# monahand1023/imageclust

Measured on AMD Instinct MI355X. Metric: images/sec (embed+Ward), higher is better.
Workload: dtype bf16; 1 GPU; the metric's size (configs[2]'s N=100000) on 1 GPU: 100000 synthetic 224x224x3 images (structured, seed 20250217; 100000 on this rank), ResNet50-v1 bf16 batch=256 -> 2048-d pooled E -> Ward min=5 max=50 (merge loop on GPU0) -> cluster ids on host; n_images_total=100000, embed_dim=2048, weights=synthetic seed 1, device=AMD Radeon Graphics (gfx950:sramecc+:xnack-)

## Files before the change

imageclust_amd/csrc/resnet.hip:

```cpp
#include "icl_common.h"
#include "jpeg_stage.h"
#include "mfma_tile.h"

#include <algorithm>
#include <cmath>
#include <chrono>
#include <condition_variable>
#include <cstring>
#include <new>
#include <thread>
#include <type_traits>
#include <vector>

#define ICL_MAX_LANES 4

struct conv_args {
    const void *X;
    const void *Wt;
    void *Y;
    const void *R;
    const float *scale;
    const float *shift;
    const void *zero;
    int B, H, W, Cin, Ho, Wo, Cout, KH, KW, stride, pad, relu;
// ... 1142 lines not shown
            ICL_HIP(ctx, hipMemcpy(*dst, t.data(), n * 2, hipMemcpyHostToDevice));
        } else if (prec == ICL_PREC_BF16X3) {
            std::vector<uint16_t> t(2 * n);
            host_split32(src, n, t.data());
            ICL_HIP(ctx, hipMemcpy(*dst, t.data(), n * 4, hipMemcpyHostToDevice));
        } else {
            ICL_HIP(ctx, hipMemcpy(*dst, src, n * 4, hipMemcpyHostToDevice));
        }
        return ICL_OK;
    };
    void *dx = nullptr, *dw = nullptr, *dr = nullptr, *dy = nullptr, *dz = nullptr;
    float *dsc = nullptr, *dsh = nullptr;
    int rc = to_dev(x, nx, &dx);
    if (!rc && (hipMalloc(&dz, 256) != hipSuccess || hipMemset(dz, 0, 256) != hipSuccess)) rc = icl_fail(ctx, ICL_ERR_NOMEM, "icl_conv2d_fused: zero page");
    if (!rc) rc = to_dev(wp.data(), nw, &dw);
    if (!rc && residual) rc = to_dev(residual, ny, &dr);
    if (!rc) rc = upload(ctx, (void **)&dsc, scale, (size_t)Cout * 4);
    if (!rc) rc = upload(ctx, (void **)&dsh, shift, (size_t)Cout * 4);
    if (!rc && hipMalloc(&dy, ny * es) != hipSuccess) rc = icl_fail(ctx, ICL_ERR_NOMEM, "icl_conv2d_fused: output alloc");
    if (!rc) {
        conv_args a;
        a.X = dx; a.Wt = dw; a.Y = dy; a.R = dr; a.scale = dsc; a.shift = dsh; a.zero = dz;
        a.X2 = nullptr; a.H2 = a.W2 = a.Cin2 = a.stride2 = 0;
        a.B = B; a.H = a.W = H; a.Cin = Cin; a.Ho = a.Wo = Ho; a.Cout = Cout; a.KH = a.KW = k; a.stride = stride; a.pad = pad;
        a.relu = relu; a.M = (int64_t)B * Ho * Ho; a.K = k * k * Cin;
        rc = launch_conv_prec(ctx, prec, a);
    }
    if (!rc) {
        hipError_t e = hipStreamSynchronize(ctx->stream);
        if (e == hipSuccess) {
            if (prec == ICL_PREC_BF16) {
                std::vector<uint16_t> t(ny);
                e = hipMemcpy(t.data(), dy, ny * 2, hipMemcpyDeviceToHost);
                for (size_t i = 0; i < ny; ++i) y[i] = host_from_bf16(t[i]);
            } else if (prec == ICL_PREC_BF16X3) {
                std::vector<uint16_t> t(2 * ny);
                e = hipMemcpy(t.data(), dy, ny * 4, hipMemcpyDeviceToHost);
                host_join32(t.data(), ny, y);
            } else {
                e = hipMemcpy(y, dy, ny * 4, hipMemcpyDeviceToHost);
            }
        }
        if (e != hipSuccess) rc = icl_fail(ctx, ICL_ERR_HIP, "icl_conv2d_fused: %s", hipGetErrorString(e));
    }
    for (void *q : {dx, dw, dr, dy, dz, (void *)dsc, (void *)dsh})
        if (q) (void)hipFree(q);
    icl_prof_collect(ctx);
    return rc;
}

static int launch_conv_fused_ds(icl_ctx *ctx, int prec, const conv_layer &c3, const conv_layer &ds, const void *t2, const void *x, void *y, int B)
{
    conv_args a;
    a.X = t2;
    a.Wt = c3.wfused[prec];
    a.Y = y;
    a.R = nullptr;
    a.scale = ctx->model->ones;
    a.shift = c3.shift_fused;
    a.zero = ctx->model->zero;
    a.B = B;
    a.relu = 1;
    a.Cout = c3.rec.cout;
    a.H = a.W = a.Ho = a.Wo = c3.rec.hout;
    a.Cin = c3.rec.cin;
    a.KH = a.KW = 1;
    a.stride = 1;
    a.pad = 0;
    a.X2 = x;
    a.H2 = a.W2 = ds.rec.hin;
    a.Cin2 = ds.rec.cin;
    a.stride2 = ds.rec.stride;
    a.M = (int64_t)B * a.Ho * a.Wo;
    a.K = a.Cin + a.Cin2;
    const int bk = prec == ICL_PREC_BF16 ? BF16::BK : F32::BK;
    if (a.Cin % bk || a.Cin2 % bk || a.Cout % 128) return icl_fail(ctx, ICL_ERR_UNSUPPORTED, "fused downsample shape not supported");
    return launch_conv_prec(ctx, prec, a);
}

static int fuse_mask()
{
    static const int m = [] {
        const char *e = getenv("ICL_FUSE");
        return e ? atoi(e) : 15;
    }();
    return m;
}

template <typename T>
static void launch_stem_pool(icl_ctx *ctx, int prec, const uint8_t *d_img, int B, void *pooled, hipStream_t strm)
{
    icl_model *m = ctx->model;
    if (prec == ICL_PREC_BF16 && (fuse_mask() & 8)) {
        const conv_layer &L0 = m->conv[0];
        icl_prof_scope ps(ctx, ICL_K_CONV64, 2.0 * (double)B * 112 * 112 * 64 * 147, 0.0);
        const int nunits = B * SP_STRIPS;
        const int per_cu = std::max<int>(1, std::min<int>(5, (int)((size_t)160 * 1024 / stem2_lds_bytes())));
        const unsigned grid = (unsigned)std::min<int64_t>(nunits, (int64_t)per_cu * ctx->prop.multiProcessorCount);
        hipLaunchKernelGGL(stem2_pool_kernel, dim3(grid), dim3(256), stem2_lds_bytes(), strm, d_img, (const uint16_t *)L0.wfold, L0.shift, (uint16_t *)pooled, nunits);
        return;
    }
    constexpr bool SPLIT = is_x3<T>::value;
    typedef typename std::conditional<SPLIT, F32, T>::type TS;
    icl_lds_optin(ctx, (const void *)stem_pool_kernel<TS, SPLIT>, (int)stem_pool_lds_bytes<TS>());
    conv_args a;
    const conv_layer &L = m->conv[0];
    a.X = nullptr; a.Wt = L.w[SPLIT ? ICL_PREC_FP32 : prec]; a.Y = pooled; a.R = nullptr; a.scale = L.scale; a.shift = L.shift; a.zero = m->zero;
    a.B = B; a.H = a.W = 224; a.Cin = 3; a.Ho = a.Wo = 112; a.Cout = 64; a.KH = a.KW = 7; a.stride = 2; a.pad = 3; a.relu = 1;
    a.M = (int64_t)B * 112 * 112; a.K = STEM_K; a.gx = B * SP_STRIPS * SP_TILES; a.gy = 1;
    a.X2 = nullptr; a.H2 = a.W2 = a.Cin2 = a.stride2 = 0;
    icl_prof_scope ps(ctx, ICL_K_CONV64, 2.0 * (double)a.M * 64 * 147, 0.0);
    const int nunits = B * SP_STRIPS;
    const int per_cu = std::max<int>(1, (int)((size_t)160 * 1024 / stem_pool_lds_bytes<TS>()));
    const unsigned grid = (unsigned)std::min<int64_t>(nunits, (int64_t)per_cu * ctx->prop.multiProcessorCount);
    hipLaunchKernelGGL((stem_pool_kernel<TS, SPLIT>), dim3(grid), dim3(256), stem_pool_lds_bytes<TS>(), strm, d_img, a, nunits);
}

static int launch_bneck56(icl_ctx *ctx, const conv_layer &c1, const conv_layer &c2, const conv_layer &c3, const conv_layer *ds, const void *x, void *y,
                          int B, hipStream_t strm)
{
    bneck_args a;
    a.X = (const uint16_t *)x;
    a.Y = (uint16_t *)y;
    a.W1 = (const uint16_t *)c1.wfold;
    a.W2 = (const uint16_t *)c2.wfold;
    a.W3 = (const uint16_t *)(ds ? c3.wfused[ICL_PREC_BF16] : c3.wfold);
    a.sh1 = c1.shift; a.sh2 = c2.shift;
    a.sh3 = ds ? c3.shift_fused : c3.shift;
    a.B = B; a.H = c2.rec.hin; a.W = c2.rec.hin;
    if ((int64_t)B * a.H * a.W * 512 >= (1LL << 31)) return icl_fail(ctx, ICL_ERR_UNSUPPORTED, "fused bottleneck: batch of %d images exceeds the 32-bit buffer offsets", B);
    a.nstrips = (a.W + BN56_COLS - 1) / BN56_COLS;
    a.ngroups = std::max(1, std::min(B, ctx->prop.multiProcessorCount / a.nstrips));
#ifdef BN56_TIMERS
    static unsigned long long *dbg = nullptr;
    if (!dbg) (void)hipMalloc((void **)&dbg, 16 * 8);
    a.dbg = dbg;
#endif
    const double px = (double)B * a.H * a.W;
    icl_prof_scope ps(ctx, ICL_K_CONV, 2.0 * px * (64.0 * c1.rec.cin + 64.0 * 576 + 256.0 * (ds ? 128 : 64)), 0.0);
    const dim3 grid((unsigned)(a.nstrips * a.ngroups));
    if (ds) {
        icl_lds_optin(ctx, (const void *)bneck56_kernel<true>, (int)bneck56_lds_bytes<true>());
        hipLaunchKernelGGL((bneck56_kernel<true>), grid, dim3(512), bneck56_lds_bytes<true>(), strm, a);
    } else {
        icl_lds_optin(ctx, (const void *)bneck56_kernel<false>, (int)bneck56_lds_bytes<false>());
        hipLaunchKernelGGL((bneck56_kernel<false>), grid, dim3(512), bneck56_lds_bytes<false>(), strm, a);
    }
    ICL_HIP(ctx, hipGetLastError());
#ifdef BN56_TIMERS
    if (getenv("BN56_PRINT")) {
        unsigned long long h[16];
        (void)hipStreamSynchronize(strm);
        (void)hipMemcpy(h, dbg, sizeof h, hipMemcpyDeviceToHost);
        const char *fn[8] = {"carry+conv1", "wait E", "dma+t1 epi", "wait C", "conv2+t2 epi", "wait x", "wait D", ""};
        const char *bn[8] = {"t2 reads + side wait", "ST reads + t2 MFMAs", "DMA issue", "side MFMAs + epilogue", "read-back + stores", "barrier waits", "", ""};
        const int nsteps = ((B / a.ngroups) * (a.H + 1) + 7) / 8;
        fprintf(stderr, "[bn56 %s] cycles per step (steps %d):\n  front:", ds ? "ds" : "id", nsteps);
        for (int k = 0; k < 7; ++k) fprintf(stderr, " %s %.0f |", fn[k], (double)h[k] / nsteps);
        fprintf(stderr, "\n  back :");
        for (int k = 0; k < 7; ++k) fprintf(stderr, " %s %.0f |", bn[k], (double)h[8 + k] / nsteps);
        fprintf(stderr, "\n");
    }
#endif
    return ICL_OK;
}

template <typename T>
static int forward_batch(icl_ctx *ctx, int prec, const uint8_t *d_img, int B, int head, float *d_out, int lane, hipStream_t strm)
{
    typedef typename T::elem elem;
    icl_model *m = ctx->model;
    ctx->cur_stream = strm;
    const int grid = 256 * 8;
    elem *x = (elem *)m->buf[lane][0], *t1 = (elem *)m->buf[lane][1], *t2 = (elem *)m->buf[lane][2], *ds = (elem *)m->buf[lane][3],
         *y = (elem *)m->buf[lane][4];
    if ((fuse_mask() & 1) || is_x3<T>::value) {
        launch_stem_pool<T>(ctx, prec, d_img, B, x, strm);
    } else if constexpr (!is_x3<T>::value) {
        {
            icl_lds_optin(ctx, (const void *)stem_conv_kernel<T>, (int)stem_lds_bytes<T>());
            conv_args a;
            const conv_layer &L = m->conv[0];
            a.X = nullptr; a.Wt = L.w[prec]; a.Y = y; a.R = nullptr; a.scale = L.scale; a.shift = L.shift; a.zero = m->zero;
            a.B = B; a.H = a.W = 224; a.Cin = 3; a.Ho = a.Wo = 112; a.Cout = 64; a.KH = a.KW = 7; a.stride = 2; a.pad = 3; a.relu = 1;
            a.M = (int64_t)B * 112 * 112; a.K = STEM_K; a.gx = B * 98; a.gy = 1;
            a.X2 = nullptr; a.H2 = a.W2 = a.Cin2 = a.stride2 = 0;
            icl_prof_scope ps(ctx, ICL_K_CONV64, 2.0 * (double)a.M * 64 * 147, 0.0);
            const int per_cu = std::max<int>(1, (int)((size_t)160 * 1024 / stem_lds_bytes<T>()));
            const unsigned stem_grid = (unsigned)std::min<int64_t>(a.gx, (int64_t)per_cu * ctx->prop.multiProcessorCount);
            hipLaunchKernelGGL((stem_conv_kernel<T>), dim3(stem_grid), dim3(256), stem_lds_bytes<T>(), strm, d_img, a);
        }
        {
            icl_prof_scope ps(ctx, ICL_K_EMBED_OTHER, 0.0, (double)B * (802816.0 + 200704.0) * sizeof(elem));
            hipLaunchKernelGGL((maxpool_kernel<T>), dim3(grid), dim3(256), 0, strm, y, B, 112, 64, x);
        }
    }
    int ci = 1;
    while (ci < m->nconv) {
        const conv_layer &c1 = m->conv[ci], &c2 = m->conv[ci + 1], &c3 = m->conv[ci + 2];
        const bool has_ds = c1.rec.block == 0;
        if (prec == ICL_PREC_BF16 && c1.rec.stage == 1 && (fuse_mask() & (has_ds ? 4 : 2))) {
            ICL_TRY(launch_bneck56(ctx, c1, c2, c3, has_ds ? &m->conv[ci + 3] : nullptr, x, y, B, strm));
            std::swap(x, y);
            ci += has_ds ? 4 : 3;
            continue;
        }
        ICL_TRY(launch_conv(ctx, prec, c1, x, t1, nullptr, 1, B));
        ICL_TRY(launch_conv(ctx, prec, c2, t1, t2, nullptr, 1, B));
        if (has_ds)
            ICL_TRY(launch_conv_fused_ds(ctx, prec, c3, m->conv[ci + 3], t2, x, y, B));
        else
            ICL_TRY(launch_conv(ctx, prec, c3, t2, y, x, 1, B));
        std::swap(x, y);
        ci += has_ds ? 4 : 3;
    }
    float *pooled = head == ICL_HEAD_POOLED ? d_out : m->pooled[lane];
    {
        icl_prof_scope ps(ctx, ICL_K_EMBED_OTHER, 0.0, (double)B * 49.0 * 2048.0 * (is_x3<T>::value ? 4 : sizeof(elem)));
        hipLaunchKernelGGL((avgpool_kernel<T>), dim3((unsigned)icl_ceil_div((int64_t)B * 2048, 256)), dim3(256), 0, strm, x, B, 49,
                           ICL_FEAT_DIM, pooled, (int64_t)ICL_FEAT_DIM);
    }
    if (head == ICL_HEAD_DENSE0) {
        icl_prof_scope ps(ctx, ICL_K_EMBED_OTHER, 2.0 * B * 2048.0 * 1000.0, 0.0);
        hipLaunchKernelGGL(fc_kernel, dim3((unsigned)std::min<int64_t>(icl_ceil_div((int64_t)B * ICL_FC_OUT, 4), 4096)), dim3(256), 0,
                           strm, pooled, m->fcw, m->fcb, B, ICL_FEAT_DIM, ICL_FC_OUT, d_out);
    }
    ICL_HIP(ctx, hipGetLastError());
    return ICL_OK;
}

extern "C" int icl_stem_pool(icl_ctx *ctx, int prec, const uint8_t *img, int B, float *out)
{
    if (!ctx || !img || !out || B < 1) return icl_fail(ctx, ICL_ERR_ARG, "icl_stem_pool: bad argument");
    if (!prec_ok(prec)) return icl_fail(ctx, ICL_ERR_ARG, "bad prec");
    return no_throw(ctx, "icl_stem_pool", [&]() -> int {
        std::lock_guard<std::mutex> lk(ctx->mu);
        icl_device_guard g(ctx->device);
        if (!ctx->model) return icl_fail(ctx, ICL_ERR_NOMODEL, "no model loaded (call icl_model_load_* first)");
        const size_t es = prec == ICL_PREC_BF16 ? 2 : 4, ny = (size_t)B * 56 * 56 * 64;
        uint8_t *dimg = nullptr;
        void *dy = nullptr;
        int rc = ICL_OK;
        if (hipMalloc((void **)&dimg, (size_t)B * ICL_IMG_BYTES) != hipSuccess || hipMalloc(&dy, ny * es) != hipSuccess)
            rc = icl_fail(ctx, ICL_ERR_NOMEM, "icl_stem_pool: device buffers");
        if (!rc && hipMemcpy(dimg, img, (size_t)B * ICL_IMG_BYTES, hipMemcpyHostToDevice) != hipSuccess) rc = icl_fail(ctx, ICL_ERR_HIP, "icl_stem_pool: upload");
        if (!rc) {
            if (prec == ICL_PREC_BF16) launch_stem_pool<BF16>(ctx, prec, dimg, B, dy, ctx->stream);
            else if (prec == ICL_PREC_BF16X3) launch_stem_pool<BF16X3>(ctx, prec, dimg, B, dy, ctx->stream);
            else launch_stem_pool<F32>(ctx, prec, dimg, B, dy, ctx->stream);
            hipError_t e = hipGetLastError();
            if (e == hipSuccess) e = hipStreamSynchronize(ctx->stream);
            if (e == hipSuccess) {
                if (prec == ICL_PREC_BF16) {
                    std::vector<uint16_t> t(ny);
                    e = hipMemcpy(t.data(), dy, ny * 2, hipMemcpyDeviceToHost);
                    for (size_t i = 0; i < ny; ++i) out[i] = host_from_bf16(t[i]);
                } else if (prec == ICL_PREC_BF16X3) {
                    std::vector<uint16_t> t(2 * ny);
                    e = hipMemcpy(t.data(), dy, ny * 4, hipMemcpyDeviceToHost);
                    host_join32(t.data(), ny, out);
                } else {
                    e = hipMemcpy(out, dy, ny * 4, hipMemcpyDeviceToHost);
                }
            }
            if (e != hipSuccess) rc = icl_fail(ctx, ICL_ERR_HIP, "icl_stem_pool: %s", hipGetErrorString(e));
        }
        if (dimg) (void)hipFree(dimg);
        if (dy) (void)hipFree(dy);
        icl_prof_collect(ctx);
        return rc;
    });
}

extern "C" int icl_bottleneck56(icl_ctx *ctx, const float *x, int B, int H, int W, int Cin, const float *w1, const float *sc1, const float *sh1,
                                const float *w2, const float *sc2, const float *sh2, const float *w3, const float *sc3, const float *sh3,
                                const float *wds, const float *scds, const float *shds, float *y)
{
    if (!ctx || !x || !w1 || !sc1 || !sh1 || !w2 || !sc2 || !sh2 || !w3 || !sc3 || !sh3 || !y || B < 1 || H < 1 || W < 1)
        return icl_fail(ctx, ICL_ERR_ARG, "icl_bottleneck56: bad argument");
    const bool has_ds = wds != nullptr;
    if (has_ds && (!scds || !shds)) return icl_fail(ctx, ICL_ERR_ARG, "icl_bottleneck56: downsample scale / shift missing");
    if (Cin != (has_ds ? 64 : 256)) return icl_fail(ctx, ICL_ERR_UNSUPPORTED, "icl_bottleneck56: Cin must be 256 (identity) or 64 (downsample branch)");
    if ((int64_t)B * H * W * 512 >= (1LL << 31)) return icl_fail(ctx, ICL_ERR_UNSUPPORTED, "icl_bottleneck56: tensor exceeds the kernel's 32-bit buffer offsets");
    return no_throw(ctx, "icl_bottleneck56", [&]() -> int {
        std::lock_guard<std::mutex> lk(ctx->mu);
        icl_device_guard g(ctx->device);
        const size_t nx = (size_t)B * H * W * Cin, ny = (size_t)B * H * W * 256;
        const int K3 = has_ds ? 128 : 64;
        std::vector<uint16_t> hx(nx), hw1((size_t)64 * Cin), hw2((size_t)64 * 576), hw3((size_t)256 * K3);
        for (size_t i = 0; i < nx; ++i) hx[i] = host_bf16(x[i]);
        for (size_t i = 0; i < hw1.size(); ++i) hw1[i] = host_bf16(w1[i] * sc1[i / (size_t)Cin]);
        for (int co = 0; co < 64; ++co)
            for (int c = 0; c < 64; ++c)
                for (int a = 0; a < 3; ++a)
                    for (int b = 0; b < 3; ++b) hw2[(size_t)co * 576 + ((size_t)a * 3 + b) * 64 + c] = host_bf16(w2[(((size_t)co * 64 + c) * 3 + a) * 3 + b] * sc2[co]);
        std::vector<float> h3(256);
        for (int co = 0; co < 256; ++co) {
            for (int c = 0; c < 64; ++c) hw3[(size_t)co * K3 + c] = host_bf16(w3[(size_t)co * 64 + c] * sc3[co]);
            if (has_ds)
                for (int c = 0; c < 64; ++c) hw3[(size_t)co * 128 + 64 + c] = host_bf16(wds[(size_t)co * 64 + c] * scds[co]);
            h3[co] = has_ds ? sh3[co] + shds[co] : sh3[co];
        }
        void *dx = nullptr, *dy = nullptr, *dw1 = nullptr, *dw2 = nullptr, *dw3 = nullptr, *dz = nullptr;
        float *d1h = nullptr, *d2h = nullptr, *d3h = nullptr;
        int rc = upload(ctx, &dx, hx.data(), nx * 2);
        if (!rc) rc = upload(ctx, &dw1, hw1.data(), hw1.size() * 2);
        if (!rc) rc = upload(ctx, &dw2, hw2.data(), hw2.size() * 2);
        if (!rc) rc = upload(ctx, &dw3, hw3.data(), hw3.size() * 2);
        if (!rc) rc = upload(ctx, (void **)&d1h, sh1, 64 * 4);
        if (!rc) rc = upload(ctx, (void **)&d2h, sh2, 64 * 4);
        if (!rc) rc = upload(ctx, (void **)&d3h, h3.data(), 256 * 4);
        if (!rc && hipMalloc(&dy, ny * 2) != hipSuccess) rc = icl_fail(ctx, ICL_ERR_NOMEM, "icl_bottleneck56: output alloc");
        if (!rc) {
// ... 334 lines not shown
```

imageclust_amd/csrc/resnet_fused.h:

```cpp
#pragma once
#include "mfma_tile.h"

typedef float f32x4 __attribute__((ext_vector_type(4)));

__device__ __forceinline__ f32x4 mfma16(const uint4 &a, const uint4 &b, const f32x4 &c)
{
    return __builtin_amdgcn_mfma_f32_16x16x32_bf16(__builtin_bit_cast(bf16x8_t, a), __builtin_bit_cast(bf16x8_t, b), c, 0, 0, 0);
}
typedef unsigned u32x4_t __attribute__((ext_vector_type(4)));
typedef int i32x4_t __attribute__((ext_vector_type(4)));
#define BN56_OOB 0x80000000u
__device__ __forceinline__ i32x4_t bn56_srd(const void *base, unsigned bytes)
{
    const unsigned long long a = (unsigned long long)base;
    i32x4_t r;
    r.x = (int)(unsigned)a;
    r.y = (int)(unsigned)(a >> 32);
    r.z = (int)bytes;
    r.w = 0x00020000;
    return r;
}
__device__ __forceinline__ void bload_lds16_asm(const i32x4_t &srd, unsigned voff, unsigned soff, unsigned lds_dst)
{
    unsigned keep;
// ... 257 lines not shown
#define ST2_PW 40
#define ST2_RAWW 120
static constexpr size_t stem2_lds_bytes()
{
    return (size_t)((STEM_PH * ST2_RAWW + 16 + 15) & ~15) + (size_t)(STEM_PH + 1) * ST2_PW * 8 + (size_t)128 * 128 + 2 * 16 * 128;
}

__global__ __launch_bounds__(256) void stem2_pool_kernel(const uint8_t *__restrict__ img, const uint16_t *__restrict__ W2k ,
                                                        const float *__restrict__ shift, uint16_t *__restrict__ Yg , int nunits)
{
    extern __shared__ __attribute__((aligned(16))) unsigned char smem[];
    constexpr int RAWB = (STEM_PH * ST2_RAWW + 16 + 15) & ~15;
    unsigned char *raw = smem;
    unsigned char *pbf = smem + RAWB;
    unsigned char *ptile = pbf + (STEM_PH + 1) * ST2_PW * 8;
    unsigned char *carry = ptile + 128 * 128;
    const int tid = threadIdx.x, lane = tid & 63;
    const int w = __builtin_amdgcn_readfirstlane(tid >> 6);
    const int r16 = lane & 15, q = lane >> 4;
    uint4 wr[7];
#pragma unroll
    for (int kh = 0; kh < 7; ++kh) wr[kh] = *reinterpret_cast<const uint4 *>(W2k + (size_t)(16 * w + r16) * ST2_K + 32 * kh + 8 * q);
    const float4 hf = *reinterpret_cast<const float4 *>(shift + 16 * w + 4 * q);
    const f32x4 hv = f32x4{hf.x, hf.y, hf.z, hf.w};
    const int swc = (r16 >> 1) & 7;
    const unsigned boff = (unsigned)((2 * r16 + 2 * q) * 8);
    const unsigned toff = (unsigned)(r16 * 128 + ((((2 * w + (q >> 1)) ^ swc) & 7) << 4) + 8 * (q & 1));
    constexpr int RW = ST2_RAWW / 4, NDW = STEM_PH * RW + 4, NV = (NDW + 255) / 256;
    uint32_t pv[NV];
    auto patch_fetch = [&](int unit, int t) {
        const uint8_t *ib = img + (int64_t)(unit >> 3) * (int64_t)ICL_IMG_BYTES;
        const int iy0 = t * 16 - 3, bx0 = 84 * (unit & 7) - 16;
#pragma unroll
        for (int k = 0; k < NV; ++k) {
            const int i = tid + k * 256;
            const int pr = i / RW, pc = i - pr * RW;
            const int iy = iy0 + pr, bx = bx0 + pc * 4;
            const bool ok = i < NDW && pr < STEM_PH && (unsigned)iy < 224u && (unsigned)bx < 672u;
            pv[k] = ok ? *reinterpret_cast<const uint32_t *>(ib + iy * 672 + bx) : 0u;
        }
    };
    auto patch_store = [&]() {
        uint32_t *p32 = reinterpret_cast<uint32_t *>(raw);
#pragma unroll
        for (int k = 0; k < NV; ++k) {
            const int i = tid + k * 256;
            if (i < NDW) p32[i] = pv[k];
        }
    };
    const float sc255 = (float)(1.0 / 255.0);
    auto convert = [&]() {
#pragma unroll
        for (int k = 0; k < 4; ++k) {
            const int i = tid + k * 256;
            if (i < STEM_PH * ST2_PW) {
                const int pr = i / ST2_PW, pc = i - pr * ST2_PW;
                uint2 o = make_uint2(0u, 0u);
                if (pc < 38) {
                    const int addr = pr * ST2_RAWW + pc * 3 + 1;
                    const uint32_t *w32 = reinterpret_cast<const uint32_t *>(raw + (addr & ~3));
                    const uint32_t v3 = __builtin_amdgcn_alignbyte(w32[1], w32[0], addr & 3);
                    const float r = (float)(v3 & 0xffu) * sc255, g = (float)((v3 >> 8) & 0xffu) * sc255, b = (float)((v3 >> 16) & 0xffu) * sc255;
                    o.x = (uint32_t)BF16::from_f(r) | ((uint32_t)BF16::from_f(g) << 16);
                    o.y = (uint32_t)BF16::from_f(b);
                }
                *reinterpret_cast<uint2 *>(pbf + i * 8) = o;
            }
        }
    };
    int unit = blockIdx.x, t = 0;
    if (unit >= nunits) return;
    if (tid < ST2_PW) *reinterpret_cast<uint2 *>(pbf + (STEM_PH * ST2_PW + tid) * 8) = make_uint2(0u, 0u);
    patch_fetch(unit, t);
    patch_store();
    __syncthreads();
    for (;;) {
        int nt = t + 1, nu = unit;
        if (nt == SP_TILES) {
            nt = 0;
            nu = unit + (int)gridDim.x;
        }
        const bool has_next = nu < nunits;
        convert();
        if (has_next) patch_fetch(nu, nt);
        __syncthreads();
        if (has_next) patch_store();
        f32x4 acc[8];
#pragma unroll
        for (int r = 0; r < STEM_PH; ++r) {
            const uint4 bf = *reinterpret_cast<const uint4 *>(pbf + r * (ST2_PW * 8) + boff);
#pragma unroll
            for (int m = 0; m < 8; ++m) {
                const int kh = r - 2 * m;
                if (kh >= 0 && kh < 7) acc[m] = mfma16(wr[kh], bf, kh == 0 ? hv : acc[m]);
            }
        }
        unsigned char *carry_cur = carry + (t & 1) * 2048, *carry_nxt = carry + ((t + 1) & 1) * 2048;
#pragma unroll
        for (int m = 0; m < 8; ++m) {
            uint2 o;
            o.x = pack_relu_bf16x2(acc[m][0], acc[m][1]);
            o.y = pack_relu_bf16x2(acc[m][2], acc[m][3]);
            *reinterpret_cast<uint2 *>(ptile + m * 2048 + toff) = o;
            if (m == 7) *reinterpret_cast<uint2 *>(carry_nxt + toff) = o;
        }
        __syncthreads();
        if (tid < 28 * 8) {
            const int s = unit & 7;
            const int64_t b = unit >> 3;
            const int ch = tid & 7, pix = tid >> 3, pr = pix / 7, pc = pix - 7 * pr;
            i16x2_t best[4] = {i16x2_t{0, 0}, i16x2_t{0, 0}, i16x2_t{0, 0}, i16x2_t{0, 0}};
#pragma unroll
            for (int kh = 0; kh < 3; ++kh) {
                const int rr = 2 * pr + kh;
                if (rr == 0 && t == 0) continue;
                const unsigned char *rowp = rr == 0 ? carry_cur : ptile + (rr - 1) * 2048;
#pragma unroll
                for (int kw = 0; kw < 3; ++kw) {
                    const int ci = 2 * pc + kw;
                    if (s == 0 && ci == 0) continue;
                    const uint4 rawv = *reinterpret_cast<const uint4 *>(rowp + ci * 128 + (((ch ^ (ci >> 1)) & 7) << 4));
                    best[0] = __builtin_elementwise_max(best[0], __builtin_bit_cast(i16x2_t, rawv.x));
                    best[1] = __builtin_elementwise_max(best[1], __builtin_bit_cast(i16x2_t, rawv.y));
                    best[2] = __builtin_elementwise_max(best[2], __builtin_bit_cast(i16x2_t, rawv.z));
                    best[3] = __builtin_elementwise_max(best[3], __builtin_bit_cast(i16x2_t, rawv.w));
                }
            }
            const uint4 o = make_uint4(__builtin_bit_cast(uint32_t, best[0]), __builtin_bit_cast(uint32_t, best[1]), __builtin_bit_cast(uint32_t, best[2]),
                                       __builtin_bit_cast(uint32_t, best[3]));
            *reinterpret_cast<uint4 *>(Yg + ((b * 56 + 4 * t + pr) * 56 + 7 * s + pc) * 64 + ch * 8) = o;
        }
        if (!has_next) break;
        unit = nu;
        t = nt;
        __syncthreads();
    }
}

#ifdef BN56_TIMERS
#define BN56_STAMP(k)                                                                              \
    do {                                                                                           \
        unsigned long long t__;                                                                    \
        __builtin_amdgcn_sched_barrier(0);                                                         \
        asm volatile("s_memtime %0\n\ts_waitcnt lgkmcnt(0)" : "=s"(t__)::"memory");                \
        __builtin_amdgcn_sched_barrier(0);                                                         \
        tacc[k] += t__ - tlast;                                                                    \
        tlast = t__;                                                                               \
    } while (0)
#define BN56_TIMER_DECL unsigned long long tacc[8] = {0, 0, 0, 0, 0, 0, 0, 0}, tlast = 0
#define BN56_TIMER_START asm volatile("s_memtime %0\n\ts_waitcnt lgkmcnt(0)" : "=s"(tlast)::"memory")
#define BN56_TIMER_FLUSH(role)                                                                     \
    if (p.dbg && blockIdx.x == 0 && w == 0 && lane == 0)                                            \
        for (int k__ = 0; k__ < 8; ++k__) p.dbg[(role)*8 + k__] = tacc[k__]
#else
#define BN56_STAMP(k)
#define BN56_TIMER_DECL
#define BN56_TIMER_START
#define BN56_TIMER_FLUSH(role)
#endif

struct bneck_args {
    const uint16_t *X;
    uint16_t *Y;
    const uint16_t *W1;
    const uint16_t *W2;
    const uint16_t *W3;
    const float *sh1, *sh2, *sh3;
    int B, H, W;
    int nstrips, ngroups;
#ifdef BN56_TIMERS
    unsigned long long *dbg;
#endif
};

#define BN56_COLS 14
#define BN56_T1_BYTES (11 * 16 * 128)
#define BN56_T2_BYTES (128 * 128)

template <bool DS>
static constexpr size_t bneck56_lds_bytes()
{
    return (size_t)(DS ? 1 : 4) * 128 * 128 + BN56_T1_BYTES + 2 * BN56_T2_BYTES + 4 * 8192;
}

__device__ __forceinline__ void bn56_barrier() { asm volatile("s_waitcnt lgkmcnt(0)\n\ts_barrier" ::: "memory"); }
struct bn56_row {
    int b, r, p;
    __device__ __forceinline__ void step(int VH)
    {
        ++p;
        if (++r == VH) {
            r = 0;
            ++b;
            --p;
        }
    }
};

template <bool DS>
__global__ __launch_bounds__(512, 2) void bneck56_kernel(const bneck_args p)
{
    constexpr int CIN = DS ? 64 : 256;
    constexpr int NCH = CIN / 64;
    constexpr int K3 = DS ? 128 : 64;
    extern __shared__ __attribute__((aligned(16))) unsigned char smem[];
    unsigned char *XT = smem;
    unsigned char *T1 = smem + NCH * 16384;
    unsigned char *T2 = T1 + BN56_T1_BYTES;
    const int tid = threadIdx.x, lane = tid & 63;
    const int wid = __builtin_amdgcn_readfirstlane(tid >> 6);
    const int w = wid & 3;
    const int r16 = lane & 15, q = lane >> 4;
    const int H = p.H, Wd = p.W, VH = H + 1;
    const int strip = (int)blockIdx.x % p.nstrips, grp = (int)blockIdx.x / p.nstrips;
    const int b0 = (int)(((int64_t)grp * p.B) / p.ngroups), b1 = (int)(((int64_t)(grp + 1) * p.B) / p.ngroups);
    if (b0 >= b1) return;
    const int c0 = strip * BN56_COLS;
    const int nsteps = ((b1 - b0) * VH + 7) / 8;
    const int swc = (r16 >> 1) & 7;
    unsigned xoff[2];
#pragma unroll
    for (int ks = 0; ks < 2; ++ks) xoff[ks] = (unsigned)(r16 * 128 + ((((4 * ks + q) ^ swc) & 7) << 4));

    const f32x4 zero4 = f32x4{0.f, 0.f, 0.f, 0.f};
    if (wid < 4) {
        uint4 w1r[NCH * 2], w2r[18];
#pragma unroll
        for (int kk = 0; kk < NCH * 2; ++kk) w1r[kk] = *reinterpret_cast<const uint4 *>(p.W1 + (size_t)(16 * w + r16) * CIN + 32 * kk + 8 * q);
#pragma unroll
        for (int kk = 0; kk < 18; ++kk) w2r[kk] = *reinterpret_cast<const uint4 *>(p.W2 + (size_t)(16 * w + r16) * 576 + 32 * kk + 8 * q);
        const float4 h1f = *reinterpret_cast<const float4 *>(p.sh1 + 16 * w + 4 * q), h2f = *reinterpret_cast<const float4 *>(p.sh2 + 16 * w + 4 * q);
        const f32x4 h1 = f32x4{h1f.x, h1f.y, h1f.z, h1f.w}, h2 = f32x4{h2f.x, h2f.y, h2f.z, h2f.w};
        unsigned t1off[3][2];
#pragma unroll
        for (int ks = 0; ks < 2; ++ks)
#pragma unroll
            for (int kw = 0; kw < 3; ++kw) {
                const int c = r16 + kw;
                t1off[kw][ks] = (unsigned)(c * 128 + ((((4 * ks + q) ^ (c >> 1)) & 7) << 4));
            }
        const unsigned toff = (unsigned)(r16 * 128 + ((((2 * w + (q >> 1)) ^ swc) & 7) << 4) + 8 * (q & 1));
        const bool col_in = (unsigned)(c0 - 1 + r16) < (unsigned)Wd;
        const int dcol = lane >> 3, dps = lane & 7;
        const unsigned xt_wave = __builtin_amdgcn_readfirstlane(lds_addr_of(smem) + (unsigned)w * 4096u);
        const i32x4_t xsrd = bn56_srd(p.X, (unsigned)((size_t)p.B * H * Wd * CIN * 2));
        const unsigned xrow_bytes = (unsigned)(Wd * CIN * 2);
        unsigned dvoff[2];
#pragma unroll
        for (int i = 0; i < 2; ++i) {
            const int c = 8 * i + dcol, col = c0 - 1 + c;
            dvoff[i] = (unsigned)col < (unsigned)Wd ? (unsigned)(col * CIN + ((dps ^ (c >> 1)) & 7) * 8) * 2u : BN56_OOB;
        }
        auto stage_x = [&](bn56_row t) {
#pragma unroll
            for (int rr = 0; rr < 2; ++rr) {
                const bool rok = t.b < b1 && t.r < H;
                const unsigned soff = rok ? (unsigned)t.p * xrow_bytes : 0u;
#pragma unroll
                for (int i = 0; i < 2; ++i) {
                    const unsigned vo = rok ? dvoff[i] : BN56_OOB;
#pragma unroll
                    for (int ch = 0; ch < NCH; ++ch) bload_lds16_asm(xsrd, vo, soff + (unsigned)(128 * ch), xt_wave + (unsigned)(ch * 16384 + (2 * rr + i) * 1024));
                }
                t.step(VH);
            }
        };
        bn56_row cur{b0, 0, b0 * H};
        bn56_row dma = cur;
        for (int i = 0; i < 2 * w; ++i) dma.step(VH);
        reinterpret_cast<uint4 *>(T1)[tid] = make_uint4(0, 0, 0, 0);
        stage_x(dma);
        asm volatile("s_waitcnt vmcnt(0)" ::: "memory");
        bn56_barrier();
        BN56_TIMER_DECL;
        BN56_TIMER_START;
#pragma unroll 1
        for (int j = 0; j < nsteps; ++j) {
            f32x4 a1[8];
            {
                constexpr int NU = NCH * 4;
                uint4 f[3][4];
                auto ld = [&](int u, uint4 (&d)[4]) {
                    const int kk = u >> 1, m0 = 4 * (u & 1);
#pragma unroll
                    for (int m = 0; m < 4; ++m) d[m] = *reinterpret_cast<const uint4 *>(XT + (kk >> 1) * 16384 + (m0 + m) * 2048 + xoff[kk & 1]);
                };
                ld(0, f[0]);
                ld(1, f[1]);
#pragma unroll
                for (int u = 0; u < NU; ++u) {
                    if (u + 2 < NU) ld(u + 2, f[(u + 2) % 3]);
                    __builtin_amdgcn_sched_barrier(0);
                    const int kk = u >> 1, m0 = 4 * (u & 1);
#pragma unroll
                    for (int m = 0; m < 4; ++m) a1[m0 + m] = mfma16(w1r[kk], f[u % 3][m], kk == 0 ? h1 : a1[m0 + m]);
                }
            }
            BN56_STAMP(0);
            bn56_barrier();
            BN56_STAMP(1);
            for (int i = 0; i < 8; ++i) dma.step(VH);
            if (j + 1 < nsteps) stage_x(dma);
            {
                bn56_row t = cur;
#pragma unroll
                for (int m = 0; m < 8; ++m) {
                    const bool ok = t.b < b1 && t.r < H && col_in;
                    uint2 o;
                    o.x = ok ? pack_relu_bf16x2(a1[m][0], a1[m][1]) : 0u;
                    o.y = ok ? pack_relu_bf16x2(a1[m][2], a1[m][3]) : 0u;
                    *reinterpret_cast<uint2 *>(T1 + (2 + m) * 2048 + toff) = o;
                    t.step(VH);
                }
                cur = t;
            }
            BN56_STAMP(2);
            bn56_barrier();
            BN56_STAMP(3);
            f32x4 a2[8];
            {
                uint4 f[2][3];
#pragma unroll
                for (int kw = 0; kw < 3; ++kw) f[0][kw] = *reinterpret_cast<const uint4 *>(T1 + t1off[kw][0]);
#pragma unroll
                for (int u = 0; u < 20; ++u) {
                    const int R = u >> 1, ks = u & 1;
                    if (u + 1 < 20) {
#pragma unroll
                        for (int kw = 0; kw < 3; ++kw) f[(u + 1) & 1][kw] = *reinterpret_cast<const uint4 *>(T1 + ((u + 1) >> 1) * 2048 + t1off[kw][(u + 1) & 1]);
                    }
                    __builtin_amdgcn_sched_barrier(0);
#pragma unroll
                    for (int kw = 0; kw < 3; ++kw)
#pragma unroll
                        for (int kh = 0; kh < 3; ++kh) {
                            const int m = R - kh;
                            if (m >= 0 && m < 8) a2[m] = mfma16(w2r[(kh * 3 + kw) * 2 + ks], f[u & 1][kw], (kh == 0 && kw == 0 && ks == 0) ? h2 : a2[m]);
                        }
                }
            }
            unsigned char *T2w = T2 + (j & 1) * BN56_T2_BYTES;
#pragma unroll
            for (int m = 0; m < 8; ++m) {
                uint2 o;
                o.x = pack_relu_bf16x2(a2[m][0], a2[m][1]);
                o.y = pack_relu_bf16x2(a2[m][2], a2[m][3]);
                *reinterpret_cast<uint2 *>(T2w + m * 2048 + toff) = o;
            }
            BN56_STAMP(4);
            asm volatile("s_waitcnt vmcnt(0)" ::: "memory");
            BN56_STAMP(5);
            bn56_barrier();
            BN56_STAMP(6);
            reinterpret_cast<uint4 *>(T1)[tid] = reinterpret_cast<const uint4 *>(T1 + 16384)[tid];
        }
        BN56_TIMER_FLUSH(0);
        bn56_barrier();
        bn56_barrier();
    } else {
        constexpr int NW3 = DS ? 4 : 2;
        uint4 w3r[4 * NW3];
#pragma unroll
        for (int g = 0; g < 4; ++g)
#pragma unroll
            for (int ks = 0; ks < NW3; ++ks)
                w3r[g * NW3 + ks] = *reinterpret_cast<const uint4 *>(p.W3 + (size_t)(64 * w + 16 * g + r16) * K3 + 32 * ks + 8 * q);
        uint4 sel[2];
#pragma unroll
        for (int h = 0; h < 2; ++h) {
            uint32_t e[4];
#pragma unroll
            for (int d2 = 0; d2 < 4; ++d2) e[d2] = ((8 * q + 2 * d2 == 16 * h + r16) ? 0x3F80u : 0u) | ((8 * q + 2 * d2 + 1 == 16 * h + r16) ? 0x3F800000u : 0u);
            sel[h] = make_uint4(e[0], e[1], e[2], e[3]);
        }
        f32x4 h3[4];
#pragma unroll
        for (int g = 0; g < 4; ++g) {
            const float4 t = *reinterpret_cast<const float4 *>(p.sh3 + 64 * w + 16 * g + 4 * q);
            h3[g] = f32x4{t.x, t.y, t.z, t.w};
        }
        unsigned char *ST = T2 + 2 * BN56_T2_BYTES + w * 8192, *OT = ST + 4096;
        const unsigned st_lds = __builtin_amdgcn_readfirstlane(lds_addr_of(ST));
        unsigned aoff[4];
#pragma unroll
        for (int g = 0; g < 4; ++g) aoff[g] = (unsigned)(r16 * 128 + ((((2 * g + (q >> 1)) ^ swc) & 7) << 4) + 8 * (q & 1));
        const int lcol = lane >> 3, lps = lane & 7;
        const i32x4_t xsrd = bn56_srd(p.X, (unsigned)((size_t)p.B * H * Wd * CIN * 2)), ysrd = bn56_srd(p.Y, (unsigned)((size_t)p.B * H * Wd * 256 * 2));
        const unsigned xrow_bytes = (unsigned)(Wd * CIN * 2), yrow_bytes = (unsigned)(Wd * 256 * 2);
        const unsigned xbase = (unsigned)((c0 * CIN + (DS ? 0 : 64 * w)) * 2), ybase = (unsigned)((c0 * 256 + 64 * w) * 2);
        unsigned xvoff[2], yvoff[2];
#pragma unroll
        for (int i = 0; i < 2; ++i) {
            const int c = 8 * i + lcol, chunk = (lps ^ (c >> 1)) & 7;
            const bool ok = c < BN56_COLS && c0 + c < Wd;
            xvoff[i] = ok ? (unsigned)(c * CIN + chunk * 8) * 2u : BN56_OOB;
            yvoff[i] = ok ? (unsigned)(c * 256 + chunk * 8) * 2u : BN56_OOB;
        }
        auto row_ok = [&](const bn56_row &t) { return t.b >= b0 && t.b < b1 && t.r < H; };
        auto stage_side = [&](bn56_row t) {
#pragma unroll
            for (int mm = 0; mm < 2; ++mm) {
                const bool rok = row_ok(t);
                const unsigned soff = rok ? (unsigned)t.p * xrow_bytes + xbase : 0u;
#pragma unroll
                for (int i = 0; i < 2; ++i) bload_lds16_asm(xsrd, rok ? xvoff[i] : BN56_OOB, soff, st_lds + (unsigned)((2 * mm + i) * 1024));
                t.step(VH);
            }
        };
        BN56_TIMER_DECL;
        auto quarter = [&](const unsigned char *T2q, bn56_row t0, bn56_row tnext) {
            uint4 tb[2][2], xb[2][2];
#pragma unroll
            for (int mm = 0; mm < 2; ++mm)
#pragma unroll
                for (int ks = 0; ks < 2; ++ks) tb[mm][ks] = *reinterpret_cast<const uint4 *>(T2q + mm * 2048 + xoff[ks]);
            asm volatile("s_waitcnt vmcnt(4)" ::: "memory");
            BN56_STAMP(0);
#pragma unroll
            for (int mm = 0; mm < 2; ++mm)
#pragma unroll
                for (int ks = 0; ks < 2; ++ks) xb[mm][ks] = *reinterpret_cast<const uint4 *>(ST + mm * 2048 + xoff[ks]);
            f32x4 a3[4][2];
#pragma unroll
            for (int mm = 0; mm < 2; ++mm)
#pragma unroll
                for (int g = 0; g < 4; ++g) {
                    a3[g][mm] = mfma16(w3r[g * NW3 + 0], tb[mm][0], h3[g]);
                    a3[g][mm] = mfma16(w3r[g * NW3 + 1], tb[mm][1], a3[g][mm]);
                }
            asm volatile("s_waitcnt lgkmcnt(0)" ::: "memory");
            __builtin_amdgcn_sched_barrier(0);
            BN56_STAMP(1);
            stage_side(tnext);
            BN56_STAMP(2);
#pragma unroll
            for (int mm = 0; mm < 2; ++mm)
#pragma unroll
                for (int g = 0; g < 4; ++g) {
                    if constexpr (DS) {
                        a3[g][mm] = mfma16(w3r[g * NW3 + 2], xb[mm][0], a3[g][mm]);
                        a3[g][mm] = mfma16(w3r[g * NW3 + 3], xb[mm][1], a3[g][mm]);
                    } else {
                        a3[g][mm] = mfma16(sel[g & 1], xb[mm][g >> 1], a3[g][mm]);
                    }
                }
#pragma unroll
            for (int mm = 0; mm < 2; ++mm)
#pragma unroll
                for (int g = 0; g < 4; ++g) {
                    uint2 o;
                    o.x = pack_relu_bf16x2(a3[g][mm][0], a3[g][mm][1]);
                    o.y = pack_relu_bf16x2(a3[g][mm][2], a3[g][mm][3]);
                    *reinterpret_cast<uint2 *>(OT + mm * 2048 + aoff[g]) = o;
                }
            asm volatile("s_waitcnt lgkmcnt(0)" ::: "memory");
            __builtin_amdgcn_sched_barrier(0);
            BN56_STAMP(3);
            bn56_row t = t0;
#pragma unroll
            for (int mm = 0; mm < 2; ++mm) {
                const bool rok = row_ok(t);
                const unsigned soff = rok ? (unsigned)t.p * yrow_bytes + ybase : 0u;
#pragma unroll
                for (int i = 0; i < 2; ++i) {
                    const uint4 v = *reinterpret_cast<const uint4 *>(OT + (2 * mm + i) * 1024 + lane * 16);
                    bstore16_asm(ysrd, rok ? yvoff[i] : BN56_OOB, soff, v);
                }
                t.step(VH);
            }
            BN56_STAMP(4);
        };
        bn56_row out{b0 - 1, H, b0 * H};
        bn56_barrier();
        stage_side(out);
#pragma unroll
        for (int i = 0; i < 4; ++i) bstore16_asm(ysrd, BN56_OOB, 0u, make_uint4(0, 0, 0, 0));
        bn56_barrier();
        bn56_barrier();
        bn56_barrier();
        BN56_TIMER_START;
#pragma unroll 1
        for (int j = 1; j <= nsteps; ++j) {
            const unsigned char *T2r = T2 + ((j - 1) & 1) * BN56_T2_BYTES;
            bn56_row r1 = out, r2, r3, r4;
            r1.step(VH); r1.step(VH);
            r2 = r1; r2.step(VH); r2.step(VH);
            r3 = r2; r3.step(VH); r3.step(VH);
            r4 = r3; r4.step(VH); r4.step(VH);
            quarter(T2r, out, r1);
            bn56_barrier();
            BN56_STAMP(5);
            quarter(T2r + 2 * 2048, r1, r2);
            bn56_barrier();
            BN56_STAMP(5);
            quarter(T2r + 4 * 2048, r2, r3);
            quarter(T2r + 6 * 2048, r3, r4);
            out = r4;
            if (j < nsteps) bn56_barrier();
            BN56_STAMP(5);
        }
        asm volatile("s_waitcnt vmcnt(0)" ::: "memory");
        BN56_TIMER_FLUSH(1);
    }
}
```

Baseline: 70560 images/sec.

## Halve bottleneck step to 4 rows and reuse staged input for residual side path

Shrinks each step of the fused 56x56 bottleneck kernel from 8 to 4 output rows and triple-buffers the staged input tile in LDS. The back-end waves now read the residual/downsample input straight from the front-end's staged X tiles instead of issuing their own global-to-LDS side loads. This removes a duplicate global read of the input and cuts LDS footprint per buffer. In exchange there are more steps and barriers per image and a larger conv2 halo overhead per output row, with tighter coupling between the producer and consumer waves.

```diff
diff --git a/imageclust_amd/csrc/resnet.hip b/imageclust_amd/csrc/resnet.hip
--- a/imageclust_amd/csrc/resnet.hip
+++ b/imageclust_amd/csrc/resnet.hip
@@ -1318,13 +1318,13 @@
         unsigned long long h[16];
         (void)hipStreamSynchronize(strm);
         (void)hipMemcpy(h, dbg, sizeof h, hipMemcpyDeviceToHost);
-        const char *fn[8] = {"carry+conv1", "wait E", "dma+t1 epi", "wait C", "conv2+t2 epi", "wait x", "wait D", ""};
-        const char *bn[8] = {"t2 reads + side wait", "ST reads + t2 MFMAs", "DMA issue", "side MFMAs + epilogue", "read-back + stores", "barrier waits", "", ""};
-        const int nsteps = ((B / a.ngroups) * (a.H + 1) + 7) / 8;
+        const char *fn[8] = BN56_FRONT_SEGMENTS;
+        const char *bn[8] = BN56_BACK_SEGMENTS;
+        const int nsteps = ((B / a.ngroups) * (a.H + 1) + BN56_ROWS - 1) / BN56_ROWS;
         fprintf(stderr, "[bn56 %s] cycles per step (steps %d):\n  front:", ds ? "ds" : "id", nsteps);
-        for (int k = 0; k < 7; ++k) fprintf(stderr, " %s %.0f |", fn[k], (double)h[k] / nsteps);
+        for (int k = 0; k < 8 && fn[k][0]; ++k) fprintf(stderr, " %s %.0f |", fn[k], (double)h[k] / nsteps);
         fprintf(stderr, "\n  back :");
-        for (int k = 0; k < 7; ++k) fprintf(stderr, " %s %.0f |", bn[k], (double)h[8 + k] / nsteps);
+        for (int k = 0; k < 8 && bn[k][0]; ++k) fprintf(stderr, " %s %.0f |", bn[k], (double)h[8 + k] / nsteps);
         fprintf(stderr, "\n");
     }
 #endif
diff --git a/imageclust_amd/csrc/resnet_fused.h b/imageclust_amd/csrc/resnet_fused.h
--- a/imageclust_amd/csrc/resnet_fused.h
+++ b/imageclust_amd/csrc/resnet_fused.h
@@ -433,6 +433,8 @@
 #define BN56_TIMER_FLUSH(role)                                                                     \
     if (p.dbg && blockIdx.x == 0 && w == 0 && lane == 0)                                            \
         for (int k__ = 0; k__ < 8; ++k__) p.dbg[(role)*8 + k__] = tacc[k__]
+#define BN56_FRONT_SEGMENTS {"carry+conv1", "wait E", "dma+t1 epi", "wait C", "conv2+t2 epi", "wait x", "wait D", ""}
+#define BN56_BACK_SEGMENTS {"t2 + side reads", "MFMAs + epilogue", "read-back + stores", "barrier waits", "", "", "", ""}
 #else
 #define BN56_STAMP(k)
 #define BN56_TIMER_DECL
@@ -455,13 +457,17 @@
 };
 
 #define BN56_COLS 14
-#define BN56_T1_BYTES (11 * 16 * 128)
-#define BN56_T2_BYTES (128 * 128)
+#define BN56_ROWS 4
+#define BN56_ROW_BYTES (16 * 128)
+#define BN56_XCH_BYTES (BN56_ROWS * BN56_ROW_BYTES)
+#define BN56_T1_BYTES ((2 + BN56_ROWS + 1) * BN56_ROW_BYTES)
+#define BN56_T2_BYTES (BN56_ROWS * BN56_ROW_BYTES)
+#define BN56_OT_BYTES (2 * BN56_ROW_BYTES)
 
 template <bool DS>
 static constexpr size_t bneck56_lds_bytes()
 {
-    return (size_t)(DS ? 1 : 4) * 128 * 128 + BN56_T1_BYTES + 2 * BN56_T2_BYTES + 4 * 8192;
+    return (size_t)3 * (DS ? 1 : 4) * BN56_XCH_BYTES + BN56_T1_BYTES + 2 * BN56_T2_BYTES + 4 * BN56_OT_BYTES;
 }
 
 __device__ __forceinline__ void bn56_barrier() { asm volatile("s_waitcnt lgkmcnt(0)\n\ts_barrier" ::: "memory"); }
@@ -481,12 +487,15 @@
 template <bool DS>
 __global__ __launch_bounds__(512, 2) void bneck56_kernel(const bneck_args p)
 {
+    static_assert(BN56_ROWS == 4, "the quarters below are rows {-1, 0} and {1, 2} of a 4-row step");
     constexpr int CIN = DS ? 64 : 256;
     constexpr int NCH = CIN / 64;
     constexpr int K3 = DS ? 128 : 64;
+    constexpr int RB = BN56_ROW_BYTES;
+    constexpr unsigned SLOT = NCH * BN56_XCH_BYTES;
     extern __shared__ __attribute__((aligned(16))) unsigned char smem[];
     unsigned char *XT = smem;
-    unsigned char *T1 = smem + NCH * 16384;
+    unsigned char *T1 = smem + 3 * SLOT;
     unsigned char *T2 = T1 + BN56_T1_BYTES;
     const int tid = threadIdx.x, lane = tid & 63;
     const int wid = __builtin_amdgcn_readfirstlane(tid >> 6);
@@ -497,7 +506,7 @@
     const int b0 = (int)(((int64_t)grp * p.B) / p.ngroups), b1 = (int)(((int64_t)(grp + 1) * p.B) / p.ngroups);
     if (b0 >= b1) return;
     const int c0 = strip * BN56_COLS;
-    const int nsteps = ((b1 - b0) * VH + 7) / 8;
+    const int nsteps = ((b1 - b0) * VH + BN56_ROWS - 1) / BN56_ROWS;
     const int swc = (r16 >> 1) & 7;
     unsigned xoff[2];
 #pragma unroll
@@ -523,7 +532,7 @@
         const unsigned toff = (unsigned)(r16 * 128 + ((((2 * w + (q >> 1)) ^ swc) & 7) << 4) + 8 * (q & 1));
         const bool col_in = (unsigned)(c0 - 1 + r16) < (unsigned)Wd;
         const int dcol = lane >> 3, dps = lane & 7;
-        const unsigned xt_wave = __builtin_amdgcn_readfirstlane(lds_addr_of(smem) + (unsigned)w * 4096u);
+        const unsigned xt_wave = __builtin_amdgcn_readfirstlane(lds_addr_of(smem) + (unsigned)w * (unsigned)RB);
         const i32x4_t xsrd = bn56_srd(p.X, (unsigned)((size_t)p.B * H * Wd * CIN * 2));
         const unsigned xrow_bytes = (unsigned)(Wd * CIN * 2);
         unsigned dvoff[2];
@@ -532,65 +541,62 @@
             const int c = 8 * i + dcol, col = c0 - 1 + c;
             dvoff[i] = (unsigned)col < (unsigned)Wd ? (unsigned)(col * CIN + ((dps ^ (c >> 1)) & 7) * 8) * 2u : BN56_OOB;
         }
-        auto stage_x = [&](bn56_row t) {
-#pragma unroll
-            for (int rr = 0; rr < 2; ++rr) {
-                const bool rok = t.b < b1 && t.r < H;
-                const unsigned soff = rok ? (unsigned)t.p * xrow_bytes : 0u;
-#pragma unroll
-                for (int i = 0; i < 2; ++i) {
-                    const unsigned vo = rok ? dvoff[i] : BN56_OOB;
-#pragma unroll
-                    for (int ch = 0; ch < NCH; ++ch) bload_lds16_asm(xsrd, vo, soff + (unsigned)(128 * ch), xt_wave + (unsigned)(ch * 16384 + (2 * rr + i) * 1024));
-                }
-                t.step(VH);
+        auto stage_x = [&](const bn56_row &t, unsigned slot) {
+            const bool rok = t.b < b1 && t.r < H;
+            const unsigned soff = rok ? (unsigned)t.p * xrow_bytes : 0u;
+#pragma unroll
+            for (int i = 0; i < 2; ++i) {
+                const unsigned vo = rok ? dvoff[i] : BN56_OOB;
+#pragma unroll
+                for (int ch = 0; ch < NCH; ++ch) bload_lds16_asm(xsrd, vo, soff + (unsigned)(128 * ch), xt_wave + slot + (unsigned)(ch * BN56_XCH_BYTES + i * 1024));
             }
         };
         bn56_row cur{b0, 0, b0 * H};
         bn56_row dma = cur;
-        for (int i = 0; i < 2 * w; ++i) dma.step(VH);
+        for (int i = 0; i < w; ++i) dma.step(VH);
         reinterpret_cast<uint4 *>(T1)[tid] = make_uint4(0, 0, 0, 0);
-        stage_x(dma);
+        stage_x(dma, 0u);
         asm volatile("s_waitcnt vmcnt(0)" ::: "memory");
         bn56_barrier();
+        unsigned xs = 0u;
         BN56_TIMER_DECL;
         BN56_TIMER_START;
 #pragma unroll 1
         for (int j = 0; j < nsteps; ++j) {
-            f32x4 a1[8];
+            f32x4 a1[BN56_ROWS];
             {
-                constexpr int NU = NCH * 4;
+                constexpr int NU = NCH * 2;
+                const unsigned char *Xc = XT + xs;
                 uint4 f[3][4];
-                auto ld = [&](int u, uint4 (&d)[4]) {
-                    const int kk = u >> 1, m0 = 4 * (u & 1);
-#pragma unroll
-                    for (int m = 0; m < 4; ++m) d[m] = *reinterpret_cast<const uint4 *>(XT + (kk >> 1) * 16384 + (m0 + m) * 2048 + xoff[kk & 1]);
+                auto ld = [&](int kk, uint4 (&d)[4]) {
+#pragma unroll
+                    for (int m = 0; m < 4; ++m) d[m] = *reinterpret_cast<const uint4 *>(Xc + (kk >> 1) * BN56_XCH_BYTES + m * RB + xoff[kk & 1]);
                 };
                 ld(0, f[0]);
                 ld(1, f[1]);
 #pragma unroll
-                for (int u = 0; u < NU; ++u) {
-                    if (u + 2 < NU) ld(u + 2, f[(u + 2) % 3]);
+                for (int kk = 0; kk < NU; ++kk) {
+                    if (kk + 2 < NU) ld(kk + 2, f[(kk + 2) % 3]);
                     __builtin_amdgcn_sched_barrier(0);
-                    const int kk = u >> 1, m0 = 4 * (u & 1);
-#pragma unroll
-                    for (int m = 0; m < 4; ++m) a1[m0 + m] = mfma16(w1r[kk], f[u % 3][m], kk == 0 ? h1 : a1[m0 + m]);
+#pragma unroll
+                    for (int m = 0; m < 4; ++m) a1[m] = mfma16(w1r[kk], f[kk % 3][m], kk == 0 ? h1 : a1[m]);
                 }
             }
             BN56_STAMP(0);
             bn56_barrier();
             BN56_STAMP(1);
-            for (int i = 0; i < 8; ++i) dma.step(VH);
-            if (j + 1 < nsteps) stage_x(dma);
+            for (int i = 0; i < BN56_ROWS; ++i) dma.step(VH);
+            const unsigned xn = xs + SLOT == 3 * SLOT ? 0u : xs + SLOT;
+            if (j + 1 < nsteps) stage_x(dma, xn);
             {
                 bn56_row t = cur;
 #pragma unroll
-                for (int m = 0; m < 8; ++m) {
+                for (int m = 0; m < BN56_ROWS; ++m) {
                     const bool ok = t.b < b1 && t.r < H && col_in;
                     uint2 o;
                     o.x = ok ? pack_relu_bf16x2(a1[m][0], a1[m][1]) : 0u;
                     o.y = ok ? pack_relu_bf16x2(a1[m][2], a1[m][3]) : 0u;
-                    *reinterpret_cast<uint2 *>(T1 + (2 + m) * 2048 + toff) = o;
+                    *reinterpret_cast<uint2 *>(T1 + (2 + m) * RB + toff) = o;
                     t.step(VH);
                 }
                 cur = t;
@@ -598,17 +604,18 @@
             BN56_STAMP(2);
             bn56_barrier();
             BN56_STAMP(3);
-            f32x4 a2[8];
+            f32x4 a2[BN56_ROWS];
             {
+                constexpr int NU = 2 * (BN56_ROWS + 2);
                 uint4 f[2][3];
 #pragma unroll
                 for (int kw = 0; kw < 3; ++kw) f[0][kw] = *reinterpret_cast<const uint4 *>(T1 + t1off[kw][0]);
 #pragma unroll
-                for (int u = 0; u < 20; ++u) {
+                for (int u = 0; u < NU; ++u) {
                     const int R = u >> 1, ks = u & 1;
-                    if (u + 1 < 20) {
-#pragma unroll
-                        for (int kw = 0; kw < 3; ++kw) f[(u + 1) & 1][kw] = *reinterpret_cast<const uint4 *>(T1 + ((u + 1) >> 1) * 2048 + t1off[kw][(u + 1) & 1]);
+                    if (u + 1 < NU) {
+#pragma unroll
+                        for (int kw = 0; kw < 3; ++kw) f[(u + 1) & 1][kw] = *reinterpret_cast<const uint4 *>(T1 + ((u + 1) >> 1) * RB + t1off[kw][(u + 1) & 1]);
                     }
                     __builtin_amdgcn_sched_barrier(0);
 #pragma unroll
@@ -616,24 +623,25 @@
 #pragma unroll
                         for (int kh = 0; kh < 3; ++kh) {
                             const int m = R - kh;
-                            if (m >= 0 && m < 8) a2[m] = mfma16(w2r[(kh * 3 + kw) * 2 + ks], f[u & 1][kw], (kh == 0 && kw == 0 && ks == 0) ? h2 : a2[m]);
+                            if (m >= 0 && m < BN56_ROWS) a2[m] = mfma16(w2r[(kh * 3 + kw) * 2 + ks], f[u & 1][kw], (kh == 0 && kw == 0 && ks == 0) ? h2 : a2[m]);
                         }
                 }
             }
             unsigned char *T2w = T2 + (j & 1) * BN56_T2_BYTES;
 #pragma unroll
-            for (int m = 0; m < 8; ++m) {
+            for (int m = 0; m < BN56_ROWS; ++m) {
                 uint2 o;
                 o.x = pack_relu_bf16x2(a2[m][0], a2[m][1]);
                 o.y = pack_relu_bf16x2(a2[m][2], a2[m][3]);
-                *reinterpret_cast<uint2 *>(T2w + m * 2048 + toff) = o;
+                *reinterpret_cast<uint2 *>(T2w + m * RB + toff) = o;
             }
             BN56_STAMP(4);
             asm volatile("s_waitcnt vmcnt(0)" ::: "memory");
             BN56_STAMP(5);
             bn56_barrier();
             BN56_STAMP(6);
-            reinterpret_cast<uint4 *>(T1)[tid] = reinterpret_cast<const uint4 *>(T1 + 16384)[tid];
+            reinterpret_cast<uint4 *>(T1)[tid] = reinterpret_cast<const uint4 *>(T1 + BN56_ROWS * RB)[tid];
+            xs = xn;
         }
         BN56_TIMER_FLUSH(0);
         bn56_barrier();
@@ -660,47 +668,39 @@
             const float4 t = *reinterpret_cast<const float4 *>(p.sh3 + 64 * w + 16 * g + 4 * q);
             h3[g] = f32x4{t.x, t.y, t.z, t.w};
         }
-        unsigned char *ST = T2 + 2 * BN56_T2_BYTES + w * 8192, *OT = ST + 4096;
-        const unsigned st_lds = __builtin_amdgcn_readfirstlane(lds_addr_of(ST));
+        unsigned char *OT = T2 + 2 * BN56_T2_BYTES + w * BN56_OT_BYTES;
+        const unsigned char *XS = XT + (DS ? 0 : w) * BN56_XCH_BYTES;
+        unsigned soff[2];
+#pragma unroll
+        for (int ks = 0; ks < 2; ++ks) soff[ks] = (unsigned)((r16 + 1) * 128 + ((((4 * ks + q) ^ ((r16 + 1) >> 1)) & 7) << 4));
         unsigned aoff[4];
 #pragma unroll
         for (int g = 0; g < 4; ++g) aoff[g] = (unsigned)(r16 * 128 + ((((2 * g + (q >> 1)) ^ swc) & 7) << 4) + 8 * (q & 1));
         const int lcol = lane >> 3, lps = lane & 7;
-        const i32x4_t xsrd = bn56_srd(p.X, (unsigned)((size_t)p.B * H * Wd * CIN * 2)), ysrd = bn56_srd(p.Y, (unsigned)((size_t)p.B * H * Wd * 256 * 2));
-        const unsigned xrow_bytes = (unsigned)(Wd * CIN * 2), yrow_bytes = (unsigned)(Wd * 256 * 2);
-        const unsigned xbase = (unsigned)((c0 * CIN + (DS ? 0 : 64 * w)) * 2), ybase = (unsigned)((c0 * 256 + 64 * w) * 2);
-        unsigned xvoff[2], yvoff[2];
+        const i32x4_t ysrd = bn56_srd(p.Y, (unsigned)((size_t)p.B * H * Wd * 256 * 2));
+        const unsigned yrow_bytes = (unsigned)(Wd * 256 * 2);
+        const unsigned ybase = (unsigned)((c0 * 256 + 64 * w) * 2);
+        unsigned yvoff[2];
 #pragma unroll
         for (int i = 0; i < 2; ++i) {
             const int c = 8 * i + lcol, chunk = (lps ^ (c >> 1)) & 7;
             const bool ok = c < BN56_COLS && c0 + c < Wd;
-            xvoff[i] = ok ? (unsigned)(c * CIN + chunk * 8) * 2u : BN56_OOB;
             yvoff[i] = ok ? (unsigned)(c * 256 + chunk * 8) * 2u : BN56_OOB;
         }
         auto row_ok = [&](const bn56_row &t) { return t.b >= b0 && t.b < b1 && t.r < H; };
-        auto stage_side = [&](bn56_row t) {
-#pragma unroll
-            for (int mm = 0; mm < 2; ++mm) {
-                const bool rok = row_ok(t);
-                const unsigned soff = rok ? (unsigned)t.p * xrow_bytes + xbase : 0u;
-#pragma unroll
-                for (int i = 0; i < 2; ++i) bload_lds16_asm(xsrd, rok ? xvoff[i] : BN56_OOB, soff, st_lds + (unsigned)((2 * mm + i) * 1024));
-                t.step(VH);
-            }
-        };
         BN56_TIMER_DECL;
-        auto quarter = [&](const unsigned char *T2q, bn56_row t0, bn56_row tnext) {
+        auto quarter = [&](const unsigned char *T2q, const unsigned char *S0, const unsigned char *S1, bn56_row t0) {
             uint4 tb[2][2], xb[2][2];
 #pragma unroll
             for (int mm = 0; mm < 2; ++mm)
 #pragma unroll
-                for (int ks = 0; ks < 2; ++ks) tb[mm][ks] = *reinterpret_cast<const uint4 *>(T2q + mm * 2048 + xoff[ks]);
-            asm volatile("s_waitcnt vmcnt(4)" ::: "memory");
+                for (int ks = 0; ks < 2; ++ks) tb[mm][ks] = *reinterpret_cast<const uint4 *>(T2q + mm * RB + xoff[ks]);
+#pragma unroll
+            for (int ks = 0; ks < 2; ++ks) {
+                xb[0][ks] = *reinterpret_cast<const uint4 *>(S0 + soff[ks]);
+                xb[1][ks] = *reinterpret_cast<const uint4 *>(S1 + soff[ks]);
+            }
             BN56_STAMP(0);
-#pragma unroll
-            for (int mm = 0; mm < 2; ++mm)
-#pragma unroll
-                for (int ks = 0; ks < 2; ++ks) xb[mm][ks] = *reinterpret_cast<const uint4 *>(ST + mm * 2048 + xoff[ks]);
             f32x4 a3[4][2];
 #pragma unroll
             for (int mm = 0; mm < 2; ++mm)
@@ -709,11 +709,6 @@
                     a3[g][mm] = mfma16(w3r[g * NW3 + 0], tb[mm][0], h3[g]);
                     a3[g][mm] = mfma16(w3r[g * NW3 + 1], tb[mm][1], a3[g][mm]);
                 }
-            asm volatile("s_waitcnt lgkmcnt(0)" ::: "memory");
-            __builtin_amdgcn_sched_barrier(0);
-            BN56_STAMP(1);
-            stage_side(tnext);
-            BN56_STAMP(2);
 #pragma unroll
             for (int mm = 0; mm < 2; ++mm)
 #pragma unroll
@@ -732,55 +727,50 @@
                     uint2 o;
                     o.x = pack_relu_bf16x2(a3[g][mm][0], a3[g][mm][1]);
                     o.y = pack_relu_bf16x2(a3[g][mm][2], a3[g][mm][3]);
-                    *reinterpret_cast<uint2 *>(OT + mm * 2048 + aoff[g]) = o;
+                    *reinterpret_cast<uint2 *>(OT + mm * RB + aoff[g]) = o;
                 }
             asm volatile("s_waitcnt lgkmcnt(0)" ::: "memory");
             __builtin_amdgcn_sched_barrier(0);
-            BN56_STAMP(3);
+            BN56_STAMP(1);
             bn56_row t = t0;
 #pragma unroll
             for (int mm = 0; mm < 2; ++mm) {
                 const bool rok = row_ok(t);
-                const unsigned soff = rok ? (unsigned)t.p * yrow_bytes + ybase : 0u;
+                const unsigned so = rok ? (unsigned)t.p * yrow_bytes + ybase : 0u;
 #pragma unroll
                 for (int i = 0; i < 2; ++i) {
                     const uint4 v = *reinterpret_cast<const uint4 *>(OT + (2 * mm + i) * 1024 + lane * 16);
-                    bstore16_asm(ysrd, rok ? yvoff[i] : BN56_OOB, soff, v);
+                    bstore16_asm(ysrd, rok ? yvoff[i] : BN56_OOB, so, v);
                 }
                 t.step(VH);
             }
-            BN56_STAMP(4);
+            asm volatile("s_waitcnt lgkmcnt(0)" ::: "memory");
+            BN56_STAMP(2);
         };
         bn56_row out{b0 - 1, H, b0 * H};
         bn56_barrier();
-        stage_side(out);
-#pragma unroll
-        for (int i = 0; i < 4; ++i) bstore16_asm(ysrd, BN56_OOB, 0u, make_uint4(0, 0, 0, 0));
         bn56_barrier();
         bn56_barrier();
         bn56_barrier();
+        unsigned xp = 2 * SLOT, xc = 0u;
         BN56_TIMER_START;
 #pragma unroll 1
         for (int j = 1; j <= nsteps; ++j) {
             const unsigned char *T2r = T2 + ((j - 1) & 1) * BN56_T2_BYTES;
-            bn56_row r1 = out, r2, r3, r4;
+            bn56_row r1 = out;
             r1.step(VH); r1.step(VH);
-            r2 = r1; r2.step(VH); r2.step(VH);
-            r3 = r2; r3.step(VH); r3.step(VH);
-            r4 = r3; r4.step(VH); r4.step(VH);
-            quarter(T2r, out, r1);
+            quarter(T2r, XS + xp + 3 * RB, XS + xc, out);
             bn56_barrier();
-            BN56_STAMP(5);
-            quarter(T2r + 2 * 2048, r1, r2);
             bn56_barrier();
-            BN56_STAMP(5);
-            quarter(T2r + 4 * 2048, r2, r3);
-            quarter(T2r + 6 * 2048, r3, r4);
-            out = r4;
+            BN56_STAMP(3);
+            quarter(T2r + 2 * RB, XS + xc + RB, XS + xc + 2 * RB, r1);
+            out = r1;
+            out.step(VH); out.step(VH);
+            xp = xc;
+            xc = xc + SLOT == 3 * SLOT ? 0u : xc + SLOT;
             if (j < nsteps) bn56_barrier();
-            BN56_STAMP(5);
-        }
-        asm volatile("s_waitcnt vmcnt(0)" ::: "memory");
+            BN56_STAMP(3);
+        }
         BN56_TIMER_FLUSH(1);
     }
 }
```

New measurement: 71450 images/sec, median of 6. 1.01x the previous value.
